# robotic-vision-lab/Learning-Implicitly-From-Spatial-Transformers-Network

Hardware: AMD Instinct MI355X
Metric: SDF query-points/sec (B=8, N=20k, 224^2) (higher is better)
Workload: dtype fp16

## Files before the change

### learning-implicitly-from-spatial-transformers-network_amd/csrc/gather_kernels.hip

```cpp
#include <string.h>

#include "list_common.h"
#include "point_math.h"
#include "gather_math.h"

namespace list {

template <int V>
__device__ __forceinline__ bool any_nan(const float (&a)[V]) {
  bool bad = false;
#pragma unroll
  for (int c = 0; c < V; ++c) bad = bad || (a[c] != a[c]);
  return bad;
}
__device__ __forceinline__ bool wave_any(bool x) { return __builtin_amdgcn_ballot_w64(x) != 0; }
__device__ __forceinline__ void launder(float& x) { asm volatile("" : "+v"(x)); }
__device__ __forceinline__ void launder(int& x) { asm volatile("" : "+v"(x)); }
__device__ __forceinline__ void launder(unsigned& x) { asm volatile("" : "+v"(x)); }
__device__ __forceinline__ void launder(float4& r) { launder(r.x); launder(r.y); launder(r.z); launder(r.w); }
__device__ __forceinline__ void launder(uint4& r) { launder(r.x); launder(r.y); launder(r.z); launder(r.w); }

template <typename M>
__device__ __forceinline__ void tap_fma_masked(typename M::Raw r, float w, bool dead, float (&a)[M::V]) {
  float f[M::V];
// ... 246 lines not shown
      Bz[e][1] = M::load(base, bo + oz[ke] + oy[1] + ox[2]);
      Bz[e][2] = M::load(base, bo + oz[ke] + oy[2] + ox[1]);
      Bz[e][3] = M::load(base, bo + oz[ke] + oy[2] + ox[2]);
    }
    float P[4][V];
#pragma unroll
    for (int k = 0; k < 4; ++k) plane4<M>(A[k][0], A[k][1], A[k][2], A[k][3], wyz, P[k]);
    store_wsum<FMT, V>(P, wcx, xh, xl, out_off + 0 * C, p.valid);
    store_wsum<FMT, V>(P, wmx, xh, xl, out_off + 1 * C, p.valid);
    store_wsum<FMT, V>(P, wpx, xh, xl, out_off + 2 * C, p.valid);
    plane4<M>(By[0][0], By[0][1], By[0][2], By[0][3], wxz, P[0]);
    plane4<M>(A[1][0], A[2][0], A[1][2], A[2][2], wxz, P[1]);
    plane4<M>(A[1][1], A[2][1], A[1][3], A[2][3], wxz, P[2]);
    plane4<M>(By[1][0], By[1][1], By[1][2], By[1][3], wxz, P[3]);
    store_wsum<FMT, V>(P, wmy, xh, xl, out_off + 3 * C, p.valid);
    store_wsum<FMT, V>(P, wpy, xh, xl, out_off + 4 * C, p.valid);
    plane4<M>(Bz[0][0], Bz[0][1], Bz[0][2], Bz[0][3], wxy, P[0]);
    plane4<M>(A[1][0], A[2][0], A[1][1], A[2][1], wxy, P[1]);
    plane4<M>(A[1][2], A[2][2], A[1][3], A[2][3], wxy, P[2]);
    plane4<M>(Bz[1][0], Bz[1][1], Bz[1][2], Bz[1][3], wxy, P[3]);
    store_wsum<FMT, V>(P, wmz, xh, xl, out_off + 5 * C, p.valid);
    store_wsum<FMT, V>(P, wpz, xh, xl, out_off + 6 * C, p.valid);
  }
}

__device__ __forceinline__ unsigned spread3(unsigned v) {
  v = (v | (v << 4)) & 0x0C3u;
  v = (v | (v << 2)) & 0x249u;
  return v;
}

struct SortParams { int b_first; int pixel; const float* trans_mat; int ms; float clamp_hi; };

struct SortKeys { int morton; int pixel; };

__device__ __forceinline__ SortKeys sort_keys(const GatherParams& g, const SortParams& sp, int i) {
  const int64_t gp = g.p_begin + i;
  const int b = (int)(gp / g.N);
  const int n = (int)(gp - (int64_t)b * g.N);
  const float* q = g.query + (int64_t)b * g.q_sb + (int64_t)n * g.q_sn;
  const float px = q[(int64_t)g.perm0 * g.q_sc] * g.scale;
  const float py = q[(int64_t)g.perm1 * g.q_sc] * g.scale;
  const float pz = q[(int64_t)g.perm2 * g.q_sc] * g.scale;
  const int slot = (b - sp.b_first) % kSortImages;
  SortKeys k;
  k.pixel = 0;
  if (sp.pixel) {
    const Proj pr = project(sp.trans_mat + b * 12, px, py, pz, sp.ms, 1, sp.clamp_hi);
    const int pix = pr.o00;
    const int y0 = pix / sp.ms, x0 = pix - y0 * sp.ms;
    k.pixel = slot * kSortPixCells + min(y0 * ((sp.ms + 3) / 4) + (x0 >> 2), kSortPixCells - 1);
  }
  const float pc[3] = {px, py, pz};
  unsigned c[3];
#pragma unroll
  for (int a = 0; a < 3; ++a) {
    const float v = (pc[a] + 1.f) * (0.5f * kSortCellsPerAxis);
    c[a] = (unsigned)fminf(fmaxf(v, 0.f), (float)(kSortCellsPerAxis - 1));
  }
  k.morton = slot * kSortCells + (int)(spread3(c[0]) | (spread3(c[1]) << 1) | (spread3(c[2]) << 2));
  return k;
}

__global__ __launch_bounds__(256) void k_zero_i32(int4* __restrict__ p, int n4) {
  const int i = blockIdx.x * 256 + threadIdx.x;
  if (i < n4) p[i] = make_int4(0, 0, 0, 0);
}

__device__ __forceinline__ int wave_grouped_add(int* __restrict__ bins, int key, bool active, bool want_pos) {
  const int lane = threadIdx.x & 63;
  const int k = active ? key : (-1 - lane);
  unsigned lo = 0, hi = 0;
#pragma unroll
  for (int l = 0; l < 64; ++l) {
    const int kl = __builtin_amdgcn_readlane(k, l);
    if (l < 32) lo |= (kl == k) ? (1u << l) : 0u;
    else hi |= (kl == k) ? (1u << (l - 32)) : 0u;
  }
  const unsigned below_lo = lane < 32 ? lo & ((1u << lane) - 1u) : lo;
  const unsigned below_hi = lane < 32 ? 0u : hi & ((1u << (lane - 32)) - 1u);
  const int rank = __builtin_popcount(below_lo) + __builtin_popcount(below_hi);
  const int count = __builtin_popcount(lo) + __builtin_popcount(hi);
  int base = 0;
  if (active && rank == 0) base = atomicAdd(&bins[key], count);
  if (!want_pos) return 0;
  const int first = lo ? __builtin_ctz(lo) : 32 + __builtin_ctz(hi);
  return __shfl(base, first) + rank;
}

__global__ __launch_bounds__(256) void k_sort_hist(GatherParams g, SortParams sp, int* __restrict__ keys_m,
                                                   int* __restrict__ keys_p, int* __restrict__ bins_m,
                                                   int* __restrict__ bins_p) {
  const int i = blockIdx.x * 256 + threadIdx.x;
  const bool active = i < g.n_valid;
  SortKeys k;
  k.morton = 0; k.pixel = 0;
  if (active) {
    k = sort_keys(g, sp, i);
    keys_m[i] = k.morton;
    if (sp.pixel) keys_p[i] = k.pixel;
  }
  wave_grouped_add(bins_m, k.morton, active, false);
  if (sp.pixel) wave_grouped_add(bins_p, k.pixel, active, false);
}

struct SlotBase { int base[kSortImages]; };

__global__ __launch_bounds__(1024) void k_sort_scan(int* __restrict__ bins_m, int* __restrict__ bins_p,
                                                    int nslots, SlotBase sb) {
  __shared__ int part[1024];
  const bool pix = (int)blockIdx.x >= nslots;
  const int slot = pix ? blockIdx.x - nslots : blockIdx.x;
  const int cells = pix ? kSortPixCells : kSortCells;
  const int per = cells / 1024;
  int* mine = (pix ? bins_p : bins_m) + (int64_t)slot * cells + threadIdx.x * per;
  int c[8];
  int sum = 0;
#pragma unroll
  for (int i = 0; i < 8; ++i) { c[i] = i < per ? mine[i] : 0; sum += c[i]; }
  part[threadIdx.x] = sum;
  __syncthreads();
  for (int off = 1; off < 1024; off <<= 1) {
    const int v = (int)threadIdx.x >= off ? part[threadIdx.x - off] : 0;
    __syncthreads();
    part[threadIdx.x] += v;
    __syncthreads();
  }
  int run = sb.base[slot] + part[threadIdx.x] - sum;
#pragma unroll
  for (int i = 0; i < 8; ++i)
    if (i < per) { mine[i] = run; run += c[i]; }
}

__global__ __launch_bounds__(256) void k_sort_scatter(int n_valid, const int* __restrict__ keys_m,
                                                      const int* __restrict__ keys_p, int* __restrict__ bins_m,
                                                      int* __restrict__ bins_p, int* __restrict__ order,
                                                      int* __restrict__ row_of, int* __restrict__ order_img) {
  const int i = blockIdx.x * 256 + threadIdx.x;
  const bool active = i < n_valid;
  const int pos = wave_grouped_add(bins_m, active ? keys_m[i] : 0, active, true);
  if (active) order[pos] = i;
  if (order_img) {
    const int pp = wave_grouped_add(bins_p, active ? keys_p[i] : 0, active, true);
    if (active) { row_of[i] = pos; order_img[pp] = i; }
  }
}

hipError_t launch_sort_points(const GatherParams& g, const ListQueryArgs& a, const SortBuffers& sb,
                              hipStream_t s) {
  SortParams sp;
  sp.b_first = (int)(g.p_begin / g.N);
  const bool img = a.percep_feat == nullptr && sb.order_img != nullptr &&
                   a.map_size * ((a.map_size + 3) / 4) <= kSortPixCells;
  sp.pixel = img ? 1 : 0; sp.trans_mat = a.trans_mat; sp.ms = a.map_size; sp.clamp_hi = a.clamp_hi;
  const int64_t b_last = (g.p_begin + g.n_valid - 1) / g.N;
  const int nslots = (int)((b_last - sp.b_first + 1 < kSortImages) ? (b_last - sp.b_first + 1) : kSortImages);
  int* bins_m = sb.bins;
  int* bins_p = sb.bins + (size_t)nslots * kSortCells;
  const size_t nbins = (size_t)nslots * (kSortCells + (img ? kSortPixCells : 0));
  SlotBase base;
  int cnt[kSortImages] = {0};
  const int64_t p_end = g.p_begin + g.n_valid;
  for (int64_t b = sp.b_first; b <= b_last; ++b) {
    const int64_t lo = b * g.N > g.p_begin ? b * g.N : g.p_begin;
    const int64_t hi = (b + 1) * g.N < p_end ? (b + 1) * g.N : p_end;
    cnt[(b - sp.b_first) % kSortImages] += (int)(hi - lo);
  }
  int run = 0;
  for (int i = 0; i < kSortImages; ++i) { base.base[i] = run; run += cnt[i]; }
  const unsigned nb = (unsigned)((g.n_valid + 255) / 256);
  GatherParams raw = g;
  raw.order = nullptr;
  int* keys_m = sb.keys;
  LIST_LAUNCH(k_zero_i32, dim3((unsigned)((nbins / 4 + 255) / 256)), dim3(256), 0, s, 0, (int4*)sb.bins,
              (int)(nbins / 4));
  hipError_t e = hipGetLastError();
  if (e != hipSuccess) return e;
  hipLaunchKernelGGL(k_sort_hist, dim3(nb), dim3(256), 0, s, raw, sp, keys_m, sb.keys2, bins_m, bins_p);
  hipLaunchKernelGGL(k_sort_scan, dim3(img ? 2 * nslots : nslots), dim3(1024), 0, s, bins_m, bins_p, nslots, base);
  hipLaunchKernelGGL(k_sort_scatter, dim3(nb), dim3(256), 0, s, g.n_valid, keys_m, sb.keys2, bins_m, bins_p,
                     sb.order, img ? sb.row_of : nullptr, img ? sb.order_img : nullptr);
  return hipGetLastError();
}

struct ImgPoint { Proj pr; int row; int b; int valid; };

template <typename M>
__device__ __forceinline__ void reduce_proj_exact(const typename M::Raw (&v)[4], const Proj& pr, float (&r)[M::V]) {
#pragma unroll
  for (int c = 0; c < M::V; ++c) r[c] = 0.f;
  tap_fma_masked<M>(v[0], pr.w00, pr.dead & 1, r); tap_fma_masked<M>(v[1], pr.w01, (pr.dead >> 1) & 1, r);
  tap_fma_masked<M>(v[2], pr.w10, (pr.dead >> 2) & 1, r); tap_fma_masked<M>(v[3], pr.w11, (pr.dead >> 3) & 1, r);
}

template <int FMT, int F16, int OUT32 = 0>
__global__ __launch_bounds__(256) void k_gather_img(GatherParams g, const void* __restrict__ img_map,
                                                    const float* __restrict__ trans_mat, int ms,
                                                    int Ct, float clamp_hi, int col_off, int kept) {
  using M = MapT<F16>;
  using Raw = typename M::Raw;
  __shared__ ImgPoint ipt[kGatherRows];
  const int blk = xcd_contiguous_block(blockIdx.x, gridDim.x);
  if (threadIdx.x < kGatherRows) {
    int row = blk * kGatherRows + threadIdx.x;
    Pt p;
    if (g.order_img) {
      p.valid = row < g.n_valid;
      const int pt = p.valid ? g.order_img[row] : 0;
      const int64_t gp = g.p_begin + pt;
      p.b = (int)(gp / g.N);
      const int n = (int)(gp - (int64_t)p.b * g.N);
      const float* q = g.query + (int64_t)p.b * g.q_sb + (int64_t)n * g.q_sn;
      p.x = q[(int64_t)g.perm0 * g.q_sc] * g.scale;
      p.y = q[(int64_t)g.perm1 * g.q_sc] * g.scale;
      p.z = q[(int64_t)g.perm2 * g.q_sc] * g.scale;
      if (p.valid) row = g.row_of[pt];
// ... 457 lines not shown
```

### learning-implicitly-from-spatial-transformers-network_amd/csrc/list_common.h

```cpp
#pragma once

#include <hip/hip_runtime.h>
#include <hip/hip_ext.h>
#include <stdint.h>
#include <stdlib.h>

#include "list_hip.h"

namespace list {

inline int any_order() {
  static const int flag = [] {
    const char* e = getenv("LIST_LAUNCH_IN_ORDER");
    return (e && e[0] && !(e[0] == '0' && e[1] == 0)) ? 0 : (int)hipExtAnyOrderLaunch;
  }();
  return flag;
}
#define LIST_LAUNCH(kernel, grid, block, lds, s, order, ...) \
  hipExtLaunchKernelGGL(kernel, grid, block, lds, s, nullptr, nullptr, (order), __VA_ARGS__)

template <bool FP16, typename V>
__device__ __forceinline__ void x_store(const V& v, V* p) {
  if (FP16) *p = v;
  else __builtin_nontemporal_store(v, p);
// ... 215 lines not shown
  const size_t b2 = (size_t)H3 * H2 * wgrad_nominal_splits(H3, H2);
  if (b1 > big) big = b1;
  if (b2 > big) big = b2;
  return big * 4;
}
inline BwdWorkspace bwd_workspace_layout(int64_t rows, int Kp, int H1, int H2, int H3, bool fp16) {
  BwdWorkspace w;
  size_t o = 0;
  auto take = [&](size_t bytes) { size_t r = o; o = align_up(o + bytes, 256); return r; };
  w.scale = take(16);
  w.dz3_hi = take((size_t)rows * H3 * 2); w.dz3_lo = take((size_t)rows * H3 * 2);
  w.dz2_hi = take((size_t)rows * H2 * 2); w.dz2_lo = take((size_t)rows * H2 * 2);
  w.dz1_hi = take((size_t)rows * H1 * 2); w.dz1_lo = take((size_t)rows * H1 * 2);
  w.dx = take((size_t)rows * Kp * (fp16 ? 2 : 4));
  w.slab = take(wgrad_slab_bytes(Kp, H1, H2, H3));
  const int hmax = H1 > H2 ? (H1 > H3 ? H1 : H3) : (H2 > H3 ? H2 : H3);
  w.colsum = take((size_t)((rows + kColsumRows - 1) / kColsumRows) * hmax * 4);
  w.recs = take((size_t)rows * 32);
  w.vs_keys = take((size_t)rows * 8 * 4);
  w.vs_bins = take((size_t)4194304 * 4);
  w.vs_sums = take(1024 * 4);
  w.vs_recs = take((size_t)rows * LIST_N_STENCIL * 16);
  w.img_heavy_bytes = img_heavy_bytes(rows, Kp);
  w.img_heavy = take(w.img_heavy_bytes);
  w.total = o;
  return w;
}

constexpr int kSortCellsPerAxis = 16;
constexpr int kSortCells = kSortCellsPerAxis * kSortCellsPerAxis * kSortCellsPerAxis;
constexpr int kSortImages = kSortImagesC;
constexpr int kSortPixCells = kSortPixCellsC;
constexpr int kSortBins = (kSortCells + kSortPixCells) * kSortImages;

constexpr int kH3 = 256;
struct Workspace {
  size_t x_hi, x_lo, h1_hi, h1_lo, h2_hi, h2_lo;
  size_t h3_hi, h3_lo;
  size_t order, keys, bins;
  size_t order_img, row_of, keys2;
  size_t nan_tiles;
  size_t total;
};
inline size_t workspace_row_bytes(int Kp, int H1, int H2) {
  return (size_t)2 * 2 * ((size_t)Kp + H1 + H2 + kH3) + 21;
}
inline size_t workspace_fixed_bytes() { return (size_t)kSortBins * 4 + 17 * 256; }
inline Workspace workspace_layout(int64_t rows, int Kp, int H1, int H2) {
  Workspace w;
  size_t o = 0;
  auto take = [&](size_t bytes) { size_t r = o; o = align_up(o + bytes, 256); return r; };
  w.x_hi = take((size_t)rows * Kp * 2); w.x_lo = take((size_t)rows * Kp * 2);
  w.h1_hi = take((size_t)rows * H1 * 2); w.h1_lo = take((size_t)rows * H1 * 2);
  w.h2_hi = take((size_t)rows * H2 * 2); w.h2_lo = take((size_t)rows * H2 * 2);
  w.h3_hi = take((size_t)rows * kH3 * 2); w.h3_lo = take((size_t)rows * kH3 * 2);
  w.order = take((size_t)rows * 4); w.keys = take((size_t)rows * 4);
  w.order_img = take((size_t)rows * 4); w.row_of = take((size_t)rows * 4);
  w.keys2 = take((size_t)rows * 4);
  w.bins = take((size_t)kSortBins * 4);
  w.nan_tiles = take((size_t)(rows / kRowTile + 1) * 4);
  w.total = o;
  return w;
}

struct GatherParams {
  const float* query; int64_t q_sb, q_sn, q_sc;
// ... 146 lines not shown
```

### learning-implicitly-from-spatial-transformers-network_amd/csrc/point_math.h

```cpp
#pragma once

#include "list_common.h"

namespace list {

struct Pt { float x, y, z; int b; bool valid; };

__device__ __forceinline__ Pt load_point(const GatherParams& g, int row) {
  Pt p;
  p.valid = row < g.n_valid;
  const int64_t gp = g.p_begin + (p.valid ? (g.order ? g.order[row] : row) : 0);
  p.b = (int)(gp / g.N);
  const int n = (int)(gp - (int64_t)p.b * g.N);
  const float* q = g.query + (int64_t)p.b * g.q_sb + (int64_t)n * g.q_sn;
  p.x = q[(int64_t)g.perm0 * g.q_sc] * g.scale;
  p.y = q[(int64_t)g.perm1 * g.q_sc] * g.scale;
  p.z = q[(int64_t)g.perm2 * g.q_sc] * g.scale;
  return p;
}

struct Axis { int i0; int has1; float w0, w1; };
__device__ __forceinline__ Axis axis_setup(float c, int size) {
  float v = ((c + 1.f) * 0.5f) * (float)(size - 1);
  v = (v != v) ? (float)(size - 1) : fminf((float)(size - 1), fmaxf(v, 0.f));
// ... 10 lines not shown

__device__ __forceinline__ Taps make_taps(float x, float y, float z, int C, int D, int H, int W) {
  const Axis ax = axis_setup(x, W), ay = axis_setup(y, H), az = axis_setup(z, D);
  const int o000 = ((az.i0 * H + ay.i0) * W + ax.i0) * C;
  const int sx = ax.has1 ? C : 0;
  const int sy = ay.has1 ? W * C : 0;
  const int sz = az.has1 ? H * W * C : 0;
  Taps t;
  t.o[0] = o000;           t.o[1] = o000 + sx;
  t.o[2] = o000 + sy;      t.o[3] = o000 + sy + sx;
  t.o[4] = o000 + sz;      t.o[5] = o000 + sz + sx;
  t.o[6] = o000 + sz + sy; t.o[7] = o000 + sz + sy + sx;
  t.w[0] = ax.w0 * ay.w0 * az.w0; t.w[1] = ax.w1 * ay.w0 * az.w0;
  t.w[2] = ax.w0 * ay.w1 * az.w0; t.w[3] = ax.w1 * ay.w1 * az.w0;
  t.w[4] = ax.w0 * ay.w0 * az.w1; t.w[5] = ax.w1 * ay.w0 * az.w1;
  t.w[6] = ax.w0 * ay.w1 * az.w1; t.w[7] = ax.w1 * ay.w1 * az.w1;
  t.dead = (ax.has1 ? 0 : 0xAA) | (ay.has1 ? 0 : 0xCC) | (az.has1 ? 0 : 0xF0);
  return t;
}

template <int J>
__device__ __forceinline__ void stencil_point(const Pt& p, float& x, float& y, float& z) {
  x = p.x + (J == 1 ? -kDisp : J == 2 ? kDisp : 0.f);
  y = p.y + (J == 3 ? -kDisp : J == 4 ? kDisp : 0.f);
  z = p.z + (J == 5 ? -kDisp : J == 6 ? kDisp : 0.f);
}

struct Proj { int o00, o01, o10, o11; float w00, w01, w10, w11; int dead; };

__device__ __forceinline__ float clamp_keep_nan(float v, float hi) {
  return (v != v) ? v : fminf(fmaxf(v, 0.f), hi);
}

__device__ __forceinline__ Proj project(const float* __restrict__ T, float px, float py, float pz,
                                        int ms, int Ct, float clamp_hi) {
  float X = px * T[0], Y = px * T[1], Z = px * T[2];
  X = fmaf(py, T[3], X); Y = fmaf(py, T[4], Y); Z = fmaf(py, T[5], Z);
  X = fmaf(pz, T[6], X); Y = fmaf(pz, T[7], Y); Z = fmaf(pz, T[8], Z);
  X = X + T[9]; Y = Y + T[10]; Z = Z + T[11];
  const float den = Z + 1e-8f;
  float u = clamp_keep_nan(__fdiv_rn(X, den), clamp_hi);
  float v = clamp_keep_nan(__fdiv_rn(Y, den), clamp_hi);
  const float half = (float)(ms - 1) * 0.5f;
  const float gx = __fdiv_rn(u - half, half), gy = __fdiv_rn(v - half, half);
  const float ix = (gx + 1.f) * half, iy = (gy + 1.f) * half;
  const float fx = floorf(ix), fy = floorf(iy);
  const float wx1 = ix - fx, wx0 = (fx + 1.f) - ix;
  const float wy1 = iy - fy, wy0 = (fy + 1.f) - iy;
  const int x0 = min(max((int)fx, 0), ms - 1), y0 = min(max((int)fy, 0), ms - 1);
  const int x1 = min(x0 + 1, ms - 1), y1 = min(y0 + 1, ms - 1);
  Proj r;
  const bool x1_out = !(fx + 1.f <= (float)(ms - 1)), y1_out = !(fy + 1.f <= (float)(ms - 1));
  const bool x0_out = !(fx >= 0.f && fx <= (float)(ms - 1)), y0_out = !(fy >= 0.f && fy <= (float)(ms - 1));
  r.dead = ((x0_out || y0_out) ? 1 : 0) | ((x1_out || y0_out) ? 2 : 0) | ((x0_out || y1_out) ? 4 : 0) |
           ((x1_out || y1_out) ? 8 : 0);
  r.o00 = (y0 * ms + x0) * Ct; r.o01 = (y0 * ms + x1) * Ct;
  r.o10 = (y1 * ms + x0) * Ct; r.o11 = (y1 * ms + x1) * Ct;
  r.w00 = wx0 * wy0; r.w01 = wx1 * wy0; r.w10 = wx0 * wy1; r.w11 = wx1 * wy1;
  if ((r.dead & 1) && r.w00 == r.w00) r.w00 = 0.f;
  if ((r.dead & 2) && r.w01 == r.w01) r.w01 = 0.f;
  if ((r.dead & 4) && r.w10 == r.w10) r.w10 = 0.f;
  if ((r.dead & 8) && r.w11 == r.w11) r.w11 = 0.f;
  return r;
}

struct RowProjRec { int64_t base; int dx, dy; float w00, w01, w10, w11; int valid, pad_[3]; };

__device__ __forceinline__ RowProjRec row_proj_rec(const GatherParams& g, const float* __restrict__ trans_mat, int ms,
                                                   int Ct, float clamp_hi, int row) {
  const Pt pt = load_point(g, row);
  const Proj q = project(trans_mat + pt.b * 12, pt.x, pt.y, pt.z, ms, Ct, clamp_hi);
  RowProjRec r;
  r.base = (int64_t)pt.b * ms * ms * Ct + q.o00;
  r.dx = q.o01 - q.o00; r.dy = q.o10 - q.o00;
  r.w00 = q.w00; r.w01 = q.w01; r.w10 = q.w10; r.w11 = q.w11;
  r.valid = (pt.valid ? 1 : 0) | (q.dead << 1);
  r.pad_[0] = r.pad_[1] = r.pad_[2] = 0;
  return r;
}

}
```

### learning-implicitly-from-spatial-transformers-network_amd/hip.py

```python
import ctypes as C
import os
import threading

import torch

_HERE = os.path.dirname(os.path.abspath(__file__))
LIB_PATH = os.environ.get("LIST_HIP_LIB") or os.path.join(_HERE, "csrc", "liblist_hip.so")

N_IMG_LEVELS = 5
N_VOX_LEVELS = 6
PREC_BF16X3 = 0
PREC_BF16 = 1
PREC_FP16 = 2
PRECISIONS = {"bf16x3": PREC_BF16X3, "bf16": PREC_BF16, "fp16": PREC_FP16}
MAP_F32, MAP_F16 = 0, 1
MAP_DTYPES = {"f32": MAP_F32, "f16": MAP_F16}


def map_dtype_for(precision):
    return "f16" if precision in ("fp16", PREC_FP16) else "f32"


class ListMap2D(C.Structure):
    _fields_ = [("data", C.c_void_p), ("C", C.c_int32), ("H", C.c_int32), ("W", C.c_int32),
# ... 36 lines not shown
                ("workspace", C.c_void_p), ("workspace_bytes", C.c_size_t),
                ("precision", C.c_int32),
                ("stage_events", C.POINTER(C.c_void_p)), ("no_sort", C.c_int32),
                ("stage_event_sets", C.c_int32), ("percep_proj", C.c_void_p), ("no_activations", C.c_int32),
                ("no_fused_fc0", C.c_int32), ("img_proj", C.c_int32), ("img_kept_C", C.c_int32)]


class ListMlpGrads(C.Structure):
    _fields_ = [("w0", C.c_void_p), ("b0", C.c_void_p), ("w1", C.c_void_p), ("b1", C.c_void_p),
                ("w2", C.c_void_p), ("b2", C.c_void_p), ("w3", C.c_void_p), ("b3", C.c_void_p)]


class ListQueryGradArgs(C.Structure):
    _fields_ = [("fwd", C.POINTER(ListQueryArgs)), ("grad_sdf", C.c_void_p),
                ("packed_mlp_bwd", C.c_void_p), ("mlp", ListMlpGrads),
                ("grad_img_map", C.c_void_p), ("grad_trans_mat", C.c_void_p),
                ("grad_vox", ListVoxLevel * N_VOX_LEVELS),
                ("workspace", C.c_void_p), ("workspace_bytes", C.c_size_t),
                ("stage_events", C.POINTER(C.c_void_p)), ("vox_adjoint", C.c_int32),
                ("grad_percep_feat", C.c_void_p), ("gpf_sb", C.c_int64), ("gpf_sc", C.c_int64),
                ("gpf_sn", C.c_int64), ("aux_streams", C.c_void_p * 3),
                ("grad_img_levels", C.POINTER(ListMap2D)), ("grad_img_map_dtype", C.c_int32)]


VOX_ADJOINT = {"auto": 0, "scatter": 1, "gather": 2}
N_BWD_STAGES = 11
BWD_STAGE_NAMES = ("head", "wgrad_fc2", "dgrad_fc2", "wgrad_fc1", "dgrad_fc1", "dgrad_fc0", "wgrad_fc0",
                   "scatter_vox", "img_map_grad", "trans_mat_grad")

N_STAGES = 13
STAGE_VOX0, STAGE_IMG = 2, 7
STAGE_NAMES = ("sort_points", "gather_vox_l1", "gather_vox_l2", "gather_vox_l3", "gather_vox_l4",
               "gather_vox_l5", "gather_img", "gather_tail", "fc_0", "exact_redo", "fc_1", "fc_2_out")


class ListPoolArgs(C.Structure):
    _fields_ = [("B", C.c_int32), ("N", C.c_int32),
                ("pc", C.c_void_p), ("p_sb", C.c_int64), ("p_sn", C.c_int64), ("p_sc", C.c_int64),
                ("trans_mat", C.c_void_p),
                ("img_map", C.c_void_p), ("img_dtype", C.c_int32), ("map_size", C.c_int32),
                ("img_C", C.c_int32), ("clamp_hi", C.c_float),
                ("out", C.c_void_p)]


class ListPoolGradArgs(C.Structure):
    _fields_ = [("fwd", C.POINTER(ListPoolArgs)), ("grad_out", C.c_void_p), ("g_sb", C.c_int64),
                ("g_sc", C.c_int64), ("g_sn", C.c_int64), ("grad_img_map", C.c_void_p),
                ("grad_trans_mat", C.c_void_p), ("workspace", C.c_void_p), ("workspace_bytes", C.c_size_t)]


class ListQueryPlan(C.Structure):
    _fields_ = [("rows_per_chunk", C.c_int64), ("chunks", C.c_int32), ("fused_tail", C.c_int32),
                ("fc0_k", C.c_int32), ("box_levels", C.c_int32), ("fused_fc0", C.c_int32),
                ("img_proj", C.c_int32)]


EXPORTS = {
    "list_img_map_bytes": (C.c_size_t, [C.POINTER(ListMap2D), C.c_int32, C.c_int32, C.c_int32]),
    "list_prep_img_maps": (C.c_int, [C.POINTER(ListMap2D), C.c_int32, C.c_int32, C.c_int32, C.c_void_p,
                                     C.c_size_t, C.c_void_p]),
    "list_vox_pack_bytes": (C.c_size_t, [C.POINTER(ListMap3D), C.c_int32, C.c_int32]),
    "list_prep_vox_maps": (C.c_int, [C.POINTER(ListMap3D), C.c_int32, C.c_int32, C.c_void_p, C.c_size_t,
                                     C.POINTER(ListVoxLevel), C.c_void_p]),
    "list_percep_proj_bytes": (C.c_size_t, [C.c_int32, C.c_int32, C.c_int32, C.c_int32]),
    "list_percep_proj_scratch_bytes": (C.c_size_t, [C.c_int32, C.c_int32, C.c_int32, C.c_int32]),
    "list_prep_percep_proj": (C.c_int, [C.c_void_p, C.c_int32, C.c_int32, C.c_int32, C.POINTER(C.c_int32), C.c_int32,
# ... 705 lines not shown
```

### learning-implicitly-from-spatial-transformers-network_amd/csrc/gemm_kernels.hip

```cpp
#include <type_traits>

#include "list_common.h"
#include "mfma_common.h"
#include "point_math.h"
#include "gather_math.h"

namespace list {

constexpr int BM = 256, BN = 256;
constexpr int kLdsBytes = 131072;
constexpr int kProjRecBytes = BM * (int)sizeof(RowProjRec);

template <int TERMS> struct Pipe {
  static constexpr int kPlanes = TERMS == 3 ? 4 : 2;
  static constexpr int BK = TERMS == 3 ? 32 : 64;
  static constexpr int kRowBytes = BK * 2;
  static constexpr int kPlaneBytes = BM * kRowBytes;
  static constexpr int kStageBytes = kPlanes * kPlaneBytes;
  static constexpr int kStages = kLdsBytes / kStageBytes;
  static constexpr int kAhead = kStages - 1;
  static constexpr int kRowsPerPiece = 1024 / kRowBytes;
  static constexpr int kPiecesPerWave = BM / kRowsPerPiece / 8;
  static constexpr int kLoadsPerStage = kPiecesPerWave * kPlanes;
  static constexpr int kWOff = (TERMS == 3 ? 2 : 1) * kPlaneBytes;
// ... 491 lines not shown
        const float4 b0 = *(const float4*)(p.bias + col_base + c8), b1 = *(const float4*)(p.bias + col_base + c8 + 4);
        const float bb[8] = {b0.x, b0.y, b0.z, b0.w, b1.x, b1.y, b1.z, b1.w};
        float o[8];
#pragma unroll
        for (int e = 0; e < 8; ++e) o[e] = relu_nan(v[e] + bb[e]);
        store8_planes<FP16>(p.out_hi, p.out_lo, (row_base + r) * p.ldo + col_base + c8, o);
      });
    }
    __syncthreads();
    float* red = (float*)smem;
    if (col_in == 0) {
#pragma unroll
      for (int i = 0; i < 8; ++i)
#pragma unroll
        for (int e = 0; e < 4; ++e) red[wn * 256 + wm * 128 + i * 16 + row_in + e] = part[i][e];
    }
    __syncthreads();
    if (threadIdx.x < 256) {
      const int row = m0 + threadIdx.x;
      if (row < p.n_valid) {
        const int rl = threadIdx.x;
        p.sdf[p.order ? p.order[row] : row] =
            ((red[rl] + red[256 + rl]) + (red[512 + rl] + red[768 + rl])) + p.b3[0];
      }
    }
  }
}

__device__ __forceinline__ int a_quarter_row(int q, int half) { return (q >> 3) * 128 + half * 64 + (q & 7) * 8; }
__device__ __forceinline__ int w_quarter_row(int q, int half) { return (q >> 2) * 64 + half * 32 + (q & 3) * 8; }

constexpr int kLead = 4;
constexpr int kPpMinK = 512;

template <int EPI, int FP16, bool S16, int X3 = 0>
__global__ __launch_bounds__(512, 2) void k_gemm_nt_pp(GemmParams p) {
  using P = Pipe<1>;
  static_assert(X3 == 0 || (S16 && !FP16), "interleaved split operands: 16x16x32 bf16 only");
  static_assert(P::BK == 64 && P::kRowBytes == 128, "single-plane pipeline");
  static_assert(EPI != EPI_RELU_SAMPLE || (S16 && FP16 && X3 == 0), "the sampling epilogue: fp16 on the 16x16x32 shape");
  __shared__ __attribute__((aligned(16))) char smem[kLdsBytes + (EPI == EPI_RELU_SAMPLE ? kProjRecBytes : 0)];
  const int lane = threadIdx.x & 63;
  const int wave = __builtin_amdgcn_readfirstlane(threadIdx.x >> 6);
  const int wm = wave >> 2, wn = wave & 3;
  const int tiles_n = p.N / BN;
  const int ntiles = (p.M / BM) * tiles_n;
  const int tile = xcd_contiguous_block(blockIdx.x, ntiles);
  int m0 = (tile / tiles_n) * BM;
  const int n0 = (tile % tiles_n) * BN;
  if (p.tile_gate && p.tile_gate[tile / tiles_n] == 0) return;
  const char* A = p.a_hi; const char* Wt = p.w_hi;
  int Kk = p.K, lda_e = p.lda ? p.lda : p.K, a_rows_e = p.a_rows ? p.a_rows : p.M;
  [[maybe_unused]] void* dx_out = p.dx;
  if constexpr (EPI == EPI_DX) {
    if (p.n_groups > 0) {
      int mt = tile / tiles_n;
      bool found = false;
#pragma unroll
      for (int i = 0; i < kGemmMaxGroups; ++i) {
        if (!found && i < p.n_groups) {
          if (mt < p.grp[i].m_tiles || i + 1 == p.n_groups) {
            A = p.grp[i].a; Wt = p.grp[i].w; dx_out = p.grp[i].out; Kk = p.grp[i].K; a_rows_e = p.grp[i].a_rows;
            lda_e = p.grp[i].lda; found = true;
          } else {
            mt -= p.grp[i].m_tiles;
          }
// ... 15 lines not shown

  constexpr int TR = S16 ? 16 : 32;
  constexpr int KS = S16 ? 2 : 4;
  constexpr int KO = S16 ? 4 : 2;
  constexpr int HA = 64 / TR, HW = 32 / TR;
  const int frow = lane & (TR - 1), fo = lane / TR;
  const int fswz = P::swz(frow);
  const int a_row_off = (wm * 128 + frow) * P::kRowBytes;
  const int w_row_off = (wn * 64 + frow) * P::kRowBytes;
  const int64_t lda = (int64_t)lda_e * (X3 ? 4 : 2);
  const int64_t ldw = (int64_t)(p.ldw ? p.ldw : p.K) * (X3 ? 4 : 2);
  const int a_last = a_rows_e - 1;
  const int nk = X3 ? Kk / 32 : Kk / P::BK;

  auto stage_quarter = [&](char* sbase, int kbyte, int quarter) {
#pragma unroll
    for (int r = 0; r < 2; ++r) {
      const int q = 2 * wave + r;
      const bool is_a = quarter == 0 || quarter == 3;
      const int row0 = is_a ? a_quarter_row(q, quarter == 3) : w_quarter_row(q, quarter == 2);
      const int row = row0 + lane / 8;
      const int chunk = (lane % 8) ^ P::swz(row);
      const char* g = (is_a ? A + (int64_t)min(m0 + row, a_last) * lda : Wt + (int64_t)(n0 + row) * ldw) + kbyte + chunk * 16;
      if ((EPI == EPI_RELU_SPLIT || EPI == EPI_RELU_SAMPLE) && is_a) glds16_nt(g, sbase + row0 * P::kRowBytes);
      else glds16(g, sbase + (is_a ? 0 : P::kWOff) + row0 * P::kRowBytes);
    }
  };
  auto frag = [&](const char* cur, int plane_off, int row_off, int blk, int ks) -> bf16x8 {
    return *(const bf16x8*)(cur + plane_off + row_off + blk * TR * P::kRowBytes + (((KO * ks + fo) ^ fswz) << 4));
  };

  const int gap_at = p.k_gap_at, gap = p.k_gap;
  auto ktb = [&](int t) { return (t + (t >= gap_at ? gap : 0)) * P::kRowBytes; };
#pragma unroll
  for (int g = 0; g < kLead; ++g)
    if (g / 4 < nk) stage_quarter(smem + ((g / 4) & 1) * P::kStageBytes, ktb(g / 4), g & 3);
  if constexpr (EPI == EPI_RELU_SAMPLE) {
    if (wm == 0)
      *((RowProjRec*)(smem + kLdsBytes) + threadIdx.x) =
          row_proj_rec(p.smp_pts, p.smp_trans_mat, p.smp_ms, p.smp_Ct, p.smp_clamp_hi, m0 + (int)threadIdx.x);
  }
  if (nk > 1) wait_vmcnt<2 * (kLead - 4)>(); else wait_vmcnt<0>();
  __builtin_amdgcn_s_barrier();
  if (wm == 1) __builtin_amdgcn_s_barrier();
  const int last_quarter = 4 * nk - 1;

  bf16x8 a[HA][KS], w[2][HW][KS];
  auto k_tile = [&](int t, auto steady) {
    constexpr bool STEADY = decltype(steady)::value;
    const char* cur = smem + (t & 1) * P::kStageBytes;
#pragma unroll
    for (int ph = 0; ph < 4; ++ph) {
      if (ph == 0 || ph == 1) {
#pragma unroll
        for (int ks = 0; ks < KS; ++ks)
#pragma unroll
          for (int b = 0; b < HW; ++b) w[ph][b][ks] = frag(cur, P::kWOff, w_row_off, ph * HW + b, ks);
      }
      if (ph == 0 || ph == 2) {
#pragma unroll
        for (int ks = 0; ks < KS; ++ks)
#pragma unroll
          for (int b = 0; b < HA; ++b) a[b][ks] = frag(cur, 0, a_row_off, (ph / 2) * HA + b, ks);
      }
      const int tt = t + (ph + kLead) / 4;
      const int sq = (ph + kLead) & 3;
      if (STEADY) {
        stage_quarter(smem + (tt & 1) * P::kStageBytes, ktb(tt), sq);
        wait_vmcnt<2 * (kLead - 2)>();
      } else {
        if (tt < nk) stage_quarter(smem + (tt & 1) * P::kStageBytes, ktb(tt), sq);
        const int beyond = last_quarter - (4 * t + ph + 2);
        if (beyond >= 4) wait_vmcnt<2 * (kLead - 2 < 4 ? kLead - 2 : 4)>();
        else if (beyond == 3) wait_vmcnt<2 * (kLead - 2 < 3 ? kLead - 2 : 3)>();
        else if (beyond == 2) wait_vmcnt<4>();
        else if (beyond == 1) wait_vmcnt<2>();
        else wait_vmcnt<0>();
      }
      __builtin_amdgcn_sched_barrier(0);
      __builtin_amdgcn_s_barrier();
      asm volatile("s_waitcnt lgkmcnt(0)" ::: "memory");
      __builtin_amdgcn_sched_barrier(0);
      __builtin_amdgcn_s_setprio(1);
      const int ih = ph < 2 ? 0 : 1, jh = (ph == 0 || ph == 3) ? 0 : 1;
#pragma unroll
      for (int ks = 0; ks < KS; ++ks)
#pragma unroll
        for (int bi = 0; bi < HA; ++bi)
#pragma unroll
          for (int bj = 0; bj < HW; ++bj) {
            auto& c = acc[ih * HA + bi][jh * HW + bj];
            if constexpr (X3 != 0) {
              if (ks == 0) {
                if constexpr (X3 == 3) {
                  c = mfma16<0>(a[bi][1], w[jh][bj][0], c);
                  c = mfma16<0>(a[bi][0], w[jh][bj][1], c);
                }
                c = mfma16<0>(a[bi][0], w[jh][bj][0], c);
              }
            } else if constexpr (S16) c = mfma16<FP16>(a[bi][ks], w[jh][bj][ks], c);
            else c = mfma<FP16>(a[bi][ks], w[jh][bj][ks], c);
          }
      __builtin_amdgcn_s_setprio(0);
      __builtin_amdgcn_sched_barrier(0);
      __builtin_amdgcn_s_barrier();
      __builtin_amdgcn_sched_barrier(0);
    }
  };
  int t = 0;
  for (; t + 3 <= nk; ++t) k_tile(t, std::true_type());
  for (; t < nk; ++t) k_tile(t, std::false_type());
  if (wm == 0) __builtin_amdgcn_s_barrier();
  if constexpr (S16) gemm_epilogue16<EPI, FP16>(p, acc, smem, m0, n0, wm, wn, wave, lane, dx_out);
  else gemm_epilogue<EPI, FP16>(p, acc, smem, m0, n0, wm, wn, wave, lane);
}

template <int TERMS, int EPI, int FP16>
__global__ __launch_bounds__(512, 2) void k_gemm_nt16(GemmParams p) {
  __shared__ __attribute__((aligned(16))) char smem[kLdsBytes];
  const int lane = threadIdx.x & 63;
  const int wave = __builtin_amdgcn_readfirstlane(threadIdx.x >> 6);
  const int wm = wave >> 2, wn = wave & 3;
  const int tiles_n = p.N / BN;
  const int ntiles = (p.M / BM) * tiles_n;
  const int tile = xcd_contiguous_block(blockIdx.x, ntiles);
  const int m0 = (tile / tiles_n) * BM, n0 = (tile % tiles_n) * BN;
  if (p.tile_gate && p.tile_gate[tile / tiles_n] == 0) return;

  f32x4v acc[8][4];
#pragma unroll
  for (int i = 0; i < 8; ++i)
#pragma unroll
    for (int j = 0; j < 4; ++j)
#pragma unroll
      for (int e = 0; e < 4; ++e) acc[i][j][e] = 0.f;

  using P = Pipe<TERMS>;
  const int frow = lane & 15, fq = lane >> 4;
  const int fswz = P::swz(frow);
  const int a_row_off = (wm * 128 + frow) * P::kRowBytes;
  const int w_row_off = (wn * 64 + frow) * P::kRowBytes;

  const int nk = p.K / P::BK;
#pragma unroll
// ... 280 lines not shown
```

Measured before the change: 89.31 million.

## Fuse point sort into single-launch block-local counting sort with LDS histograms

Replaces the four-kernel sort pipeline (zero bins, histogram with global atomics, scan, scatter) with one kernel when a size heuristic allows it. Each block owns a range of key cells for one image slot and one point partition. It recomputes keys, counts into LDS, scans locally and scatters. This removes launch overhead, the global key and bin round-trips and the global atomics, at the cost of every block re-reading all points of its slot. It also splits projection into a pixel-only helper so the pixel key avoids computing the full bilinear weights.

```diff
diff --git a/learning-implicitly-from-spatial-transformers-network_amd/csrc/gather_kernels.hip b/learning-implicitly-from-spatial-transformers-network_amd/csrc/gather_kernels.hip
--- a/learning-implicitly-from-spatial-transformers-network_amd/csrc/gather_kernels.hip
+++ b/learning-implicitly-from-spatial-transformers-network_amd/csrc/gather_kernels.hip
@@ -302,34 +302,32 @@
 
 struct SortParams { int b_first; int pixel; const float* trans_mat; int ms; float clamp_hi; };
 
-struct SortKeys { int morton; int pixel; };
-
-__device__ __forceinline__ SortKeys sort_keys(const GatherParams& g, const SortParams& sp, int i) {
-  const int64_t gp = g.p_begin + i;
-  const int b = (int)(gp / g.N);
-  const int n = (int)(gp - (int64_t)b * g.N);
+struct SortPoint { float x, y, z; };
+
+__device__ __forceinline__ SortPoint sort_point(const GatherParams& g, int b, int n) {
   const float* q = g.query + (int64_t)b * g.q_sb + (int64_t)n * g.q_sn;
-  const float px = q[(int64_t)g.perm0 * g.q_sc] * g.scale;
-  const float py = q[(int64_t)g.perm1 * g.q_sc] * g.scale;
-  const float pz = q[(int64_t)g.perm2 * g.q_sc] * g.scale;
-  const int slot = (b - sp.b_first) % kSortImages;
-  SortKeys k;
-  k.pixel = 0;
-  if (sp.pixel) {
-    const Proj pr = project(sp.trans_mat + b * 12, px, py, pz, sp.ms, 1, sp.clamp_hi);
-    const int pix = pr.o00;
-    const int y0 = pix / sp.ms, x0 = pix - y0 * sp.ms;
-    k.pixel = slot * kSortPixCells + min(y0 * ((sp.ms + 3) / 4) + (x0 >> 2), kSortPixCells - 1);
-  }
-  const float pc[3] = {px, py, pz};
-  unsigned c[3];
-#pragma unroll
-  for (int a = 0; a < 3; ++a) {
-    const float v = (pc[a] + 1.f) * (0.5f * kSortCellsPerAxis);
-    c[a] = (unsigned)fminf(fmaxf(v, 0.f), (float)(kSortCellsPerAxis - 1));
-  }
-  k.morton = slot * kSortCells + (int)(spread3(c[0]) | (spread3(c[1]) << 1) | (spread3(c[2]) << 2));
-  return k;
+  SortPoint p;
+  p.x = q[(int64_t)g.perm0 * g.q_sc] * g.scale;
+  p.y = q[(int64_t)g.perm1 * g.q_sc] * g.scale;
+  p.z = q[(int64_t)g.perm2 * g.q_sc] * g.scale;
+  return p;
+}
+
+template <bool PIX>
+__device__ __forceinline__ int sort_keys(const SortParams& sp, int b, const SortPoint& p) {
+  if constexpr (PIX) {
+    const ProjPixel pr = project_pixel(sp.trans_mat + b * 12, p.x, p.y, p.z, sp.ms, sp.clamp_hi);
+    return min(pr.y0 * ((sp.ms + 3) / 4) + (pr.x0 >> 2), kSortPixCells - 1);
+  } else {
+    const float pc[3] = {p.x, p.y, p.z};
+    unsigned c[3];
+#pragma unroll
+    for (int a = 0; a < 3; ++a) {
+      const float v = (pc[a] + 1.f) * (0.5f * kSortCellsPerAxis);
+      c[a] = (unsigned)fminf(fmaxf(v, 0.f), (float)(kSortCellsPerAxis - 1));
+    }
+    return (int)(spread3(c[0]) | (spread3(c[1]) << 1) | (spread3(c[2]) << 2));
+  }
 }
 
 __global__ __launch_bounds__(256) void k_zero_i32(int4* __restrict__ p, int n4) {
@@ -363,15 +361,18 @@
                                                    int* __restrict__ bins_p) {
   const int i = blockIdx.x * 256 + threadIdx.x;
   const bool active = i < g.n_valid;
-  SortKeys k;
-  k.morton = 0; k.pixel = 0;
+  int km = 0, kp = 0;
   if (active) {
-    k = sort_keys(g, sp, i);
-    keys_m[i] = k.morton;
-    if (sp.pixel) keys_p[i] = k.pixel;
-  }
-  wave_grouped_add(bins_m, k.morton, active, false);
-  if (sp.pixel) wave_grouped_add(bins_p, k.pixel, active, false);
+    const int64_t gp = g.p_begin + i;
+    const int b = (int)(gp / g.N);
+    const SortPoint p = sort_point(g, b, (int)(gp - (int64_t)b * g.N));
+    const int slot = (b - sp.b_first) % kSortImages;
+    km = slot * kSortCells + sort_keys<false>(sp, b, p);
+    keys_m[i] = km;
+    if (sp.pixel) { kp = slot * kSortPixCells + sort_keys<true>(sp, b, p); keys_p[i] = kp; }
+  }
+  wave_grouped_add(bins_m, km, active, false);
+  if (sp.pixel) wave_grouped_add(bins_p, kp, active, false);
 }
 
 struct SlotBase { int base[kSortImages]; };
@@ -416,6 +417,126 @@
   }
 }
 
+constexpr int kSortThreads = 1024;
+constexpr int kSortUnroll = 8;
+
+template <bool PIX, typename F>
+__device__ __forceinline__ void sort_walk(const GatherParams& g, const SortParams& sp, int slot, int n_img,
+                                          int n_from, int n_to, F&& f) {
+  const int64_t p_end = g.p_begin + g.n_valid;
+  for (int b = sp.b_first + slot; b < sp.b_first + n_img; b += kSortImages) {
+    const int64_t ib = (int64_t)b * g.N;
+    const int c_lo = (int)(ib >= g.p_begin ? 0 : g.p_begin - ib);
+    const int c_hi = (int)(ib + g.N <= p_end ? g.N : p_end - ib);
+    const int n_lo = c_lo > n_from ? c_lo : n_from, n_hi = c_hi < n_to ? c_hi : n_to;
+    const int i_off = (int)(ib - g.p_begin);
+    for (int n0 = n_lo; n0 < n_hi; n0 += kSortUnroll * kSortThreads) {
+      SortPoint p[kSortUnroll];
+#pragma unroll
+      for (int u = 0; u < kSortUnroll; ++u) {
+        const int n = n0 + u * kSortThreads + (int)threadIdx.x;
+        p[u] = sort_point(g, b, n < n_hi ? n : n_hi - 1);
+      }
+#pragma unroll
+      for (int u = 0; u < kSortUnroll; ++u) {
+        if (n0 + u * kSortThreads >= n_hi) break;
+        const int n = n0 + u * kSortThreads + (int)threadIdx.x;
+        f(i_off + n, n, sort_keys<PIX>(sp, b, p[u]), n < n_hi);
+      }
+    }
+  }
+}
+
+template <bool PIX>
+__device__ __forceinline__ void sort_role(const GatherParams& g, const SortParams& sp, const SlotBase& sb, int slot,
+                                          int n_img, int r, int part, int part_len, int* cnt, int* wave_sum,
+                                          int* below_all, int* __restrict__ bins_p, int* __restrict__ order,
+                                          int* __restrict__ row_of, int* __restrict__ order_img) {
+  constexpr int per = kSortRangeCells;
+  constexpr int items = per / kSortThreads;
+  const int c0 = r * per, n_mine = part * part_len;
+  const int tid = threadIdx.x, lane = tid & 63;
+  for (int c = tid; c < 2 * per; c += kSortThreads) cnt[c] = 0;
+  if (tid == 0) *below_all = 0;
+  __syncthreads();
+  int below = 0;
+  sort_walk<PIX>(g, sp, slot, n_img, 0, g.N, [&](int, int n, int key, bool active) {
+    if (c0 > 0) below += __builtin_popcountll(__builtin_amdgcn_ballot_w64(active && key < c0));
+    const unsigned cell = (unsigned)(key - c0);
+    if (active && cell < (unsigned)per) atomicAdd(&cnt[cell + (n < n_mine ? 0 : per)], 1);
+  });
+  if (lane == 0 && below) atomicAdd(below_all, below);
+  __syncthreads();
+  int before[items], all[items];
+  int sum = 0;
+#pragma unroll
+  for (int k = 0; k < items; ++k) {
+    before[k] = cnt[tid * items + k];
+    all[k] = before[k] + cnt[per + tid * items + k];
+    sum += all[k];
+  }
+  int inc = sum;
+#pragma unroll
+  for (int off = 1; off < 64; off <<= 1) {
+    const int v = __shfl_up(inc, off);
+    if (lane >= off) inc += v;
+  }
+  if (lane == 63) wave_sum[tid >> 6] = inc;
+  __syncthreads();
+  int run = sb.base[slot] + *below_all + inc - sum;
+  for (int w = 0; w < (tid >> 6); ++w) run += wave_sum[w];
+#pragma unroll
+  for (int k = 0; k < items; ++k) {
+    cnt[tid * items + k] = run + before[k];
+    run += all[k];
+    if (PIX && part == 0) bins_p[(int64_t)slot * kSortPixCells + c0 + tid * items + k] = run;
+  }
+  __syncthreads();
+  sort_walk<PIX>(g, sp, slot, n_img, n_mine, n_mine + part_len, [&](int i, int, int key, bool active) {
+    const unsigned cell = (unsigned)(key - c0);
+    const bool in = active && cell < (unsigned)per;
+    if (in) {
+      const int pos = atomicAdd(&cnt[cell], 1);
+      if constexpr (PIX) order_img[pos] = i;
+      else { order[pos] = i; if (row_of) row_of[i] = pos; }
+    }
+  });
+}
+
+__global__ __launch_bounds__(kSortThreads) void k_sort_points(GatherParams g, SortParams sp, SlotBase sb, int nslots,
+                                                              int n_img, int parts, int part_len,
+                                                              int* __restrict__ bins_p, int* __restrict__ order,
+                                                              int* __restrict__ row_of, int* __restrict__ order_img) {
+  __shared__ int cnt[2 * kSortRangeCells];
+  __shared__ int wave_sum[kSortThreads / 64];
+  __shared__ int below_all;
+  constexpr int ranges_m = kSortCells / kSortRangeCells, ranges_p = kSortPixCells / kSortRangeCells;
+  int role = blockIdx.x;
+  const int n_morton = nslots * parts * ranges_m;
+  const bool pix = role >= n_morton;
+  if (pix) role -= n_morton;
+  const int part = role % parts;
+  role /= parts;
+  if (pix)
+    sort_role<true>(g, sp, sb, role / ranges_p, n_img, role % ranges_p, part, part_len, cnt, wave_sum, &below_all,
+                    bins_p, order, row_of, order_img);
+  else
+    sort_role<false>(g, sp, sb, role / ranges_m, n_img, role % ranges_m, part, part_len, cnt, wave_sum, &below_all,
+                     bins_p, order, row_of, order_img);
+}
+
+static int sort_parts_for(int n_points, int groups_per_part) {
+  int parts = 1;
+  while (parts < kSortMaxParts && n_points > parts * kSortPartPoints && 2 * parts * groups_per_part <= kSortMaxGroups)
+    parts *= 2;
+  return parts;
+}
+
+static bool sort_in_one_launch(int slot_points, int chunk_points, bool both) {
+  return both ? (int64_t)75 * slot_points <= 7000 * 100 + (int64_t)21 * chunk_points
+              : (int64_t)50 * slot_points <= 6000 * 100 + (int64_t)8 * chunk_points;
+}
+
 hipError_t launch_sort_points(const GatherParams& g, const ListQueryArgs& a, const SortBuffers& sb,
                               hipStream_t s) {
   SortParams sp;
@@ -424,10 +545,8 @@
                    a.map_size * ((a.map_size + 3) / 4) <= kSortPixCells;
   sp.pixel = img ? 1 : 0; sp.trans_mat = a.trans_mat; sp.ms = a.map_size; sp.clamp_hi = a.clamp_hi;
   const int64_t b_last = (g.p_begin + g.n_valid - 1) / g.N;
-  const int nslots = (int)((b_last - sp.b_first + 1 < kSortImages) ? (b_last - sp.b_first + 1) : kSortImages);
-  int* bins_m = sb.bins;
-  int* bins_p = sb.bins + (size_t)nslots * kSortCells;
-  const size_t nbins = (size_t)nslots * (kSortCells + (img ? kSortPixCells : 0));
+  const int n_img = (int)(b_last - sp.b_first + 1);
+  const int nslots = n_img < kSortImages ? n_img : kSortImages;
   SlotBase base;
   int cnt[kSortImages] = {0};
   const int64_t p_end = g.p_begin + g.n_valid;
@@ -436,22 +555,35 @@
     const int64_t hi = (b + 1) * g.N < p_end ? (b + 1) * g.N : p_end;
     cnt[(b - sp.b_first) % kSortImages] += (int)(hi - lo);
   }
-  int run = 0;
-  for (int i = 0; i < kSortImages; ++i) { base.base[i] = run; run += cnt[i]; }
-  const unsigned nb = (unsigned)((g.n_valid + 255) / 256);
+  int run = 0, most = 0;
+  for (int i = 0; i < kSortImages; ++i) { base.base[i] = run; run += cnt[i]; most = cnt[i] > most ? cnt[i] : most; }
   GatherParams raw = g;
   raw.order = nullptr;
-  int* keys_m = sb.keys;
+  int* bins_m = sb.bins;
+  int* bins_p = sb.bins + (size_t)nslots * kSortCells;
+  if (sort_in_one_launch(most, g.n_valid, img)) {
+    const int ranges = kSortCells / kSortRangeCells + (img ? kSortPixCells / kSortRangeCells : 0);
+    const int n_most = g.N < g.n_valid ? g.N : g.n_valid;
+    const int parts = sort_parts_for(n_most, nslots * ranges);
+    const int part_len = ((g.N + parts - 1) / parts + kSortThreads - 1) / kSortThreads * kSortThreads;
+    const int groups = nslots * parts * ranges;
+    LIST_LAUNCH(k_sort_points, dim3((unsigned)groups), dim3(kSortThreads), 0, s, 0, raw, sp, base, nslots, n_img,
+                parts, part_len, bins_p, sb.order, img ? sb.row_of : nullptr, img ? sb.order_img : nullptr);
+    return hipGetLastError();
+  }
+  const size_t nbins = (size_t)nslots * (kSortCells + (img ? kSortPixCells : 0));
+  const unsigned nb = (unsigned)((g.n_valid + 255) / 256);
   LIST_LAUNCH(k_zero_i32, dim3((unsigned)((nbins / 4 + 255) / 256)), dim3(256), 0, s, 0, (int4*)sb.bins,
               (int)(nbins / 4));
   hipError_t e = hipGetLastError();
   if (e != hipSuccess) return e;
-  hipLaunchKernelGGL(k_sort_hist, dim3(nb), dim3(256), 0, s, raw, sp, keys_m, sb.keys2, bins_m, bins_p);
+  hipLaunchKernelGGL(k_sort_hist, dim3(nb), dim3(256), 0, s, raw, sp, sb.keys, sb.keys2, bins_m, bins_p);
   hipLaunchKernelGGL(k_sort_scan, dim3(img ? 2 * nslots : nslots), dim3(1024), 0, s, bins_m, bins_p, nslots, base);
-  hipLaunchKernelGGL(k_sort_scatter, dim3(nb), dim3(256), 0, s, g.n_valid, keys_m, sb.keys2, bins_m, bins_p,
+  hipLaunchKernelGGL(k_sort_scatter, dim3(nb), dim3(256), 0, s, g.n_valid, sb.keys, sb.keys2, bins_m, bins_p,
                      sb.order, img ? sb.row_of : nullptr, img ? sb.order_img : nullptr);
   return hipGetLastError();
 }
+
 
 struct ImgPoint { Proj pr; int row; int b; int valid; };
 
diff --git a/learning-implicitly-from-spatial-transformers-network_amd/csrc/list_common.h b/learning-implicitly-from-spatial-transformers-network_amd/csrc/list_common.h
--- a/learning-implicitly-from-spatial-transformers-network_amd/csrc/list_common.h
+++ b/learning-implicitly-from-spatial-transformers-network_amd/csrc/list_common.h
@@ -271,6 +271,10 @@
 constexpr int kSortImages = kSortImagesC;
 constexpr int kSortPixCells = kSortPixCellsC;
 constexpr int kSortBins = (kSortCells + kSortPixCells) * kSortImages;
+constexpr int kSortRangeCells = 4096;
+constexpr int kSortMaxParts = 8;
+constexpr int kSortPartPoints = 1024;
+constexpr int kSortMaxGroups = 256;
 
 constexpr int kH3 = 256;
 struct Workspace {
diff --git a/learning-implicitly-from-spatial-transformers-network_amd/csrc/point_math.h b/learning-implicitly-from-spatial-transformers-network_amd/csrc/point_math.h
--- a/learning-implicitly-from-spatial-transformers-network_amd/csrc/point_math.h
+++ b/learning-implicitly-from-spatial-transformers-network_amd/csrc/point_math.h
@@ -66,8 +66,10 @@
   return (v != v) ? v : fminf(fmaxf(v, 0.f), hi);
 }
 
-__device__ __forceinline__ Proj project(const float* __restrict__ T, float px, float py, float pz,
-                                        int ms, int Ct, float clamp_hi) {
+struct ProjPixel { float ix, iy, fx, fy; int x0, y0; };
+
+__device__ __forceinline__ ProjPixel project_pixel(const float* __restrict__ T, float px, float py, float pz, int ms,
+                                                   float clamp_hi) {
   float X = px * T[0], Y = px * T[1], Z = px * T[2];
   X = fmaf(py, T[3], X); Y = fmaf(py, T[4], Y); Z = fmaf(py, T[5], Z);
   X = fmaf(pz, T[6], X); Y = fmaf(pz, T[7], Y); Z = fmaf(pz, T[8], Z);
@@ -79,9 +81,19 @@
   const float gx = __fdiv_rn(u - half, half), gy = __fdiv_rn(v - half, half);
   const float ix = (gx + 1.f) * half, iy = (gy + 1.f) * half;
   const float fx = floorf(ix), fy = floorf(iy);
+  ProjPixel r;
+  r.ix = ix; r.iy = iy; r.fx = fx; r.fy = fy;
+  r.x0 = min(max((int)fx, 0), ms - 1); r.y0 = min(max((int)fy, 0), ms - 1);
+  return r;
+}
+
+__device__ __forceinline__ Proj project(const float* __restrict__ T, float px, float py, float pz,
+                                        int ms, int Ct, float clamp_hi) {
+  const ProjPixel pp = project_pixel(T, px, py, pz, ms, clamp_hi);
+  const float ix = pp.ix, iy = pp.iy, fx = pp.fx, fy = pp.fy;
+  const int x0 = pp.x0, y0 = pp.y0;
   const float wx1 = ix - fx, wx0 = (fx + 1.f) - ix;
   const float wy1 = iy - fy, wy0 = (fy + 1.f) - iy;
-  const int x0 = min(max((int)fx, 0), ms - 1), y0 = min(max((int)fy, 0), ms - 1);
   const int x1 = min(x0 + 1, ms - 1), y1 = min(y0 + 1, ms - 1);
   Proj r;
   const bool x1_out = !(fx + 1.f <= (float)(ms - 1)), y1_out = !(fy + 1.f <= (float)(ms - 1));
diff --git a/learning-implicitly-from-spatial-transformers-network_amd/hip.py b/learning-implicitly-from-spatial-transformers-network_amd/hip.py
--- a/learning-implicitly-from-spatial-transformers-network_amd/hip.py
+++ b/learning-implicitly-from-spatial-transformers-network_amd/hip.py
@@ -92,6 +92,14 @@
 STAGE_VOX0, STAGE_IMG = 2, 7
 STAGE_NAMES = ("sort_points", "gather_vox_l1", "gather_vox_l2", "gather_vox_l3", "gather_vox_l4",
                "gather_vox_l5", "gather_img", "gather_tail", "fc_0", "exact_redo", "fc_1", "fc_2_out")
+
+SORT_IMAGES, SORT_CELLS, SORT_PIX_CELLS, SORT_RANGE_CELLS = 64, 4096, 8192, 4096
+
+
+def sort_in_one_launch(slot_points, chunk_points, both_orders):
+    if both_orders:
+        return 75 * slot_points <= 700000 + 21 * chunk_points
+    return 50 * slot_points <= 600000 + 8 * chunk_points
 
 
 class ListPoolArgs(C.Structure):
```

Measured after the change: 89.92 million (median of 6 runs). Within noise of the previous version (+0.7%).

## Add two-phase k-tile schedule with deeper prefetch lead to ping-pong GEMM

Applied to the files above, without the earlier changes.

For the fp16/f32 16x16x32 variants of the ping-pong GEMM, each K tile is processed in two phases instead of four. Each phase loads one A half plus all W fragments and issues two quadrants of MFMAs, which halves the barriers per tile. The global-to-LDS prefetch lead rises from four to five quarters, with vmcnt waits retuned to match. In exchange, more W fragments stay live in registers at once, and the hand-derived wait counts are fragile at the pipeline tail.

```diff
diff --git a/learning-implicitly-from-spatial-transformers-network_amd/csrc/gemm_kernels.hip b/learning-implicitly-from-spatial-transformers-network_amd/csrc/gemm_kernels.hip
--- a/learning-implicitly-from-spatial-transformers-network_amd/csrc/gemm_kernels.hip
+++ b/learning-implicitly-from-spatial-transformers-network_amd/csrc/gemm_kernels.hip
@@ -547,6 +547,10 @@
 
 constexpr int kLead = 4;
 constexpr int kPpMinK = 512;
+
+constexpr int kLead2 = 5;
+template <int EPI, int FP16, bool S16, int X3>
+constexpr bool kTwoPhase = S16 && X3 == 0 && (EPI == EPI_F32 || (FP16 && (EPI == EPI_RELU_SPLIT || EPI == EPI_RELU_SAMPLE)));
 
 template <int EPI, int FP16, bool S16, int X3 = 0>
 __global__ __launch_bounds__(512, 2) void k_gemm_nt_pp(GemmParams p) {
@@ -628,20 +632,42 @@
 
   const int gap_at = p.k_gap_at, gap = p.k_gap;
   auto ktb = [&](int t) { return (t + (t >= gap_at ? gap : 0)) * P::kRowBytes; };
-#pragma unroll
-  for (int g = 0; g < kLead; ++g)
+  constexpr bool TWO = kTwoPhase<EPI, FP16, S16, X3>;
+  constexpr int LEAD = TWO ? kLead2 : kLead;
+#pragma unroll
+  for (int g = 0; g < LEAD; ++g)
     if (g / 4 < nk) stage_quarter(smem + ((g / 4) & 1) * P::kStageBytes, ktb(g / 4), g & 3);
   if constexpr (EPI == EPI_RELU_SAMPLE) {
     if (wm == 0)
       *((RowProjRec*)(smem + kLdsBytes) + threadIdx.x) =
           row_proj_rec(p.smp_pts, p.smp_trans_mat, p.smp_ms, p.smp_Ct, p.smp_clamp_hi, m0 + (int)threadIdx.x);
   }
-  if (nk > 1) wait_vmcnt<2 * (kLead - 4)>(); else wait_vmcnt<0>();
+  if (nk > 1) wait_vmcnt<2 * (LEAD - 4)>(); else wait_vmcnt<0>();
   __builtin_amdgcn_s_barrier();
   if (wm == 1) __builtin_amdgcn_s_barrier();
   const int last_quarter = 4 * nk - 1;
 
   bf16x8 a[HA][KS], w[2][HW][KS];
+  auto quadrant = [&](int ih, int jh) {
+#pragma unroll
+    for (int ks = 0; ks < KS; ++ks)
+#pragma unroll
+      for (int bi = 0; bi < HA; ++bi)
+#pragma unroll
+        for (int bj = 0; bj < HW; ++bj) {
+          auto& c = acc[ih * HA + bi][jh * HW + bj];
+          if constexpr (X3 != 0) {
+            if (ks == 0) {
+              if constexpr (X3 == 3) {
+                c = mfma16<0>(a[bi][1], w[jh][bj][0], c);
+                c = mfma16<0>(a[bi][0], w[jh][bj][1], c);
+              }
+              c = mfma16<0>(a[bi][0], w[jh][bj][0], c);
+            }
+          } else if constexpr (S16) c = mfma16<FP16>(a[bi][ks], w[jh][bj][ks], c);
+          else c = mfma<FP16>(a[bi][ks], w[jh][bj][ks], c);
+        }
+  };
   auto k_tile = [&](int t, auto steady) {
     constexpr bool STEADY = decltype(steady)::value;
     const char* cur = smem + (t & 1) * P::kStageBytes;
@@ -678,34 +704,70 @@
       asm volatile("s_waitcnt lgkmcnt(0)" ::: "memory");
       __builtin_amdgcn_sched_barrier(0);
       __builtin_amdgcn_s_setprio(1);
-      const int ih = ph < 2 ? 0 : 1, jh = (ph == 0 || ph == 3) ? 0 : 1;
-#pragma unroll
-      for (int ks = 0; ks < KS; ++ks)
-#pragma unroll
-        for (int bi = 0; bi < HA; ++bi)
-#pragma unroll
-          for (int bj = 0; bj < HW; ++bj) {
-            auto& c = acc[ih * HA + bi][jh * HW + bj];
-            if constexpr (X3 != 0) {
-              if (ks == 0) {
-                if constexpr (X3 == 3) {
-                  c = mfma16<0>(a[bi][1], w[jh][bj][0], c);
-                  c = mfma16<0>(a[bi][0], w[jh][bj][1], c);
-                }
-                c = mfma16<0>(a[bi][0], w[jh][bj][0], c);
-              }
-            } else if constexpr (S16) c = mfma16<FP16>(a[bi][ks], w[jh][bj][ks], c);
-            else c = mfma<FP16>(a[bi][ks], w[jh][bj][ks], c);
-          }
+      quadrant(ph < 2 ? 0 : 1, (ph == 0 || ph == 3) ? 0 : 1);
       __builtin_amdgcn_s_setprio(0);
       __builtin_amdgcn_sched_barrier(0);
       __builtin_amdgcn_s_barrier();
       __builtin_amdgcn_sched_barrier(0);
     }
   };
+  auto k_tile2 = [&](int t, auto steady) {
+    constexpr bool STEADY = decltype(steady)::value;
+    const char* cur = smem + (t & 1) * P::kStageBytes;
+#pragma unroll
+    for (int ph = 0; ph < 2; ++ph) {
+#pragma unroll
+      for (int ks = 0; ks < KS; ++ks)
+#pragma unroll
+        for (int b = 0; b < HA; ++b) a[b][ks] = frag(cur, 0, a_row_off, ph * HA + b, ks);
+      if (ph == 0) {
+        __builtin_amdgcn_sched_barrier(0);
+#pragma unroll
+        for (int jh = 0; jh < 2; ++jh)
+#pragma unroll
+          for (int ks = 0; ks < KS; ++ks)
+#pragma unroll
+            for (int b = 0; b < HW; ++b) w[jh][b][ks] = frag(cur, P::kWOff, w_row_off, jh * HW + b, ks);
+        __builtin_amdgcn_sched_barrier(0);
+      }
+#pragma unroll
+      for (int r = 0; r < 2; ++r) {
+        const int tt = t + (2 * ph + kLead2 + r) / 4;
+        const int sq = (2 * ph + kLead2 + r) & 3;
+        if (STEADY || tt < nk) stage_quarter(smem + (tt & 1) * P::kStageBytes, ktb(tt), sq);
+      }
+      if (STEADY) {
+        if (ph == 0) wait_vmcnt<6>(); else wait_vmcnt<4>();
+      } else {
+        const int k = 2 * t + ph;
+        const int fly = min(2 * k + kLead2 + 1, last_quarter) - min(4 * t + 3 + 3 * ph, last_quarter);
+        if (fly >= 3) wait_vmcnt<6>();
+        else if (fly == 2) wait_vmcnt<4>();
+        else if (fly == 1) wait_vmcnt<2>();
+        else wait_vmcnt<0>();
+      }
+      if (ph == 0) asm volatile("s_waitcnt lgkmcnt(%0)" ::"n"(2 * HW * KS < 15 ? 2 * HW * KS : 15) : "memory");
+      __builtin_amdgcn_sched_barrier(0);
+      __builtin_amdgcn_s_barrier();
+      asm volatile("s_waitcnt lgkmcnt(0)" ::: "memory");
+      __builtin_amdgcn_sched_barrier(0);
+      __builtin_amdgcn_s_setprio(1);
+      quadrant(ph, ph);
+      quadrant(ph, 1 - ph);
+      __builtin_amdgcn_s_setprio(0);
+      __builtin_amdgcn_sched_barrier(0);
+      __builtin_amdgcn_s_barrier();
+      __builtin_amdgcn_sched_barrier(0);
+    }
+  };
   int t = 0;
-  for (; t + 3 <= nk; ++t) k_tile(t, std::true_type());
-  for (; t < nk; ++t) k_tile(t, std::false_type());
+  if constexpr (TWO) {
+    for (; t + 3 <= nk; ++t) k_tile2(t, std::true_type());
+    for (; t < nk; ++t) k_tile2(t, std::false_type());
+  } else {
+    for (; t + 3 <= nk; ++t) k_tile(t, std::true_type());
+    for (; t < nk; ++t) k_tile(t, std::false_type());
+  }
   if (wm == 0) __builtin_amdgcn_s_barrier();
   if constexpr (S16) gemm_epilogue16<EPI, FP16>(p, acc, smem, m0, n0, wm, wn, wave, lane, dx_out);
   else gemm_epilogue<EPI, FP16>(p, acc, smem, m0, n0, wm, wn, wave, lane);
```

Result: no change. 88.96 million before, 89.36 million after, median of 6 (+0.4%).
